# wizyoung/YOLOv3_TensorFlow

Hardware: AMD Instinct MI355X
Metric: images/sec at 416x416 bs=32 (Darknet-53 + 3-scale head forward) (higher is better)
Workload: dtype f32

## Files before the change

yolov3_tensorflow_amd/build.py:

```python
import os
import subprocess
import sys

HERE = os.path.dirname(os.path.abspath(__file__))
CSRC = os.path.join(HERE, "csrc")
LIB = os.path.join(CSRC, "libyolo355.so")

SOURCES = [
    ("y3_abi.hip", []),
    ("y3_net_train.hip", []),
    ("y3_conv.hip", []),
    ("y3_conv_f32s.hip", []),
    ("y3_conv_bf16.hip", []),
    ("y3_conv_bf16x.hip", []),
    ("y3_conv_bf16r.hip", []),
    ("y3_conv_bf16s.hip", []),
    ("y3_conv_bf16b.hip", []),
    ("y3_conv_split.hip", []),
    ("y3_conv_wino.hip", []),
    ("y3_conv_wino44.hip", []),
    ("y3_decode.hip", ["-ffp-contract=off"]),
    ("y3_nms.hip", ["-ffp-contract=off"]),
    ("y3_ops.hip", ["-ffp-contract=off"]),
    ("y3_train.hip", ["-ffp-contract=off"]),
    ("y3_wgrad.hip", []),
    ("y3_wgrad_bf16.hip", []),
    ("y3_wgrad_wino.hip", []),
    ("y3_feed_gpu.hip", ["-ffp-contract=off"]),
    ("y3_jpeg.hip", []),
    ("y3_voc.hip", ["-ffp-contract=off"]),
    ("y3_beval.hip", ["-ffp-contract=off"]),
    ("y3_coco.hip", ["-ffp-contract=off"]),
]
COMMON = ["--offload-arch=gfx950", "-O3", "-std=c++17", "-fPIC", "-Wall", "-Wno-unused-function"]


FEED_SRC = os.path.join(CSRC, "y3_feed.cpp")
JPEG_SRC = os.path.join(CSRC, "y3_jpeg.cpp")
FEED_LIB = os.path.join(CSRC, "liby3feed.so")
FEED_FLAGS = ["-O3", "-std=c++17", "-fPIC", "-shared", "-ffp-contract=off", "-fno-fast-math", "-pthread", "-Wall",
              "-Wno-format-truncation"]


def build_feed(force=False, verbose=True):
    deps = [FEED_SRC, JPEG_SRC, os.path.join(HERE, "..", "include", "yolo355_feed.h"),
            os.path.join(HERE, "..", "include", "yolo355_jpeg.h")]
    if not force and os.path.exists(FEED_LIB) and all(os.path.getmtime(d) <= os.path.getmtime(FEED_LIB) for d in deps):
        return FEED_LIB
    tmp = FEED_LIB + ".%d.tmp" % os.getpid()
    cmd = [os.environ.get("CXX", "g++")] + FEED_FLAGS + [FEED_SRC, JPEG_SRC, "-o", tmp]
    if verbose:
        print(" ".join(cmd), flush=True)
    out = subprocess.run(cmd, stdout=subprocess.PIPE, stderr=subprocess.STDOUT)
    if out.returncode != 0:
        raise RuntimeError("building liby3feed.so failed:\n%s\n%s" % (" ".join(cmd), out.stdout.decode(errors="replace")))
    os.replace(tmp, FEED_LIB)
    return FEED_LIB


def _hipcc():
    for cand in (os.environ.get("HIPCC"), "/opt/rocm/bin/hipcc", "hipcc"):
        if cand and (os.path.isabs(cand) and os.path.exists(cand) or not os.path.isabs(cand)):
            return cand
    raise RuntimeError("hipcc not found")


def csrc_sha16():
    import hashlib
    h = hashlib.sha256()
    names = sorted(n for n in os.listdir(CSRC) if n.endswith(('.hip', '.h')))
    for path in [os.path.join(CSRC, n) for n in names] + [os.path.join(HERE, "..", "include", "yolo355.h")]:
        with open(path, 'rb') as f:
            h.update(os.path.basename(path).encode() + b'\0' + f.read())
    return h.hexdigest()[:16]


def needs_build():
    if not os.path.exists(LIB):
        return True
    t = os.path.getmtime(LIB)
    headers = sorted(n for n in os.listdir(CSRC) if n.endswith('.h'))
    deps = [os.path.join(CSRC, s) for s, _ in SOURCES] + [os.path.join(CSRC, n) for n in headers] + [
        os.path.join(HERE, "..", "include", "yolo355_jpeg.h"),
        os.path.join(HERE, "..", "include", "yolo355_feed.h"),
        os.path.join(HERE, "..", "include", "yolo355.h"),
        os.path.abspath(__file__),
    ]
    return any(os.path.getmtime(d) > t for d in deps if os.path.exists(d))


EXP_LIB = os.path.join(CSRC, "libyolo355_exp.so")
EXP_SOURCES = ("y3_conv.hip", "y3_conv_f32s.hip", "y3_conv_bf16x.hip", "y3_conv_bf16r.hip", "y3_conv_bf16s.hip", "y3_conv_bf16b.hip", "y3_conv_split.hip", "y3_conv_wino.hip", "y3_conv_wino44.hip")


def build_experiments(verbose=True):
    build(verbose=verbose)
    deps = [os.path.join(CSRC, s) for s in EXP_SOURCES] + [LIB]
    if os.path.exists(EXP_LIB) and all(os.path.getmtime(d) <= os.path.getmtime(EXP_LIB) for d in deps):
        return EXP_LIB
    hipcc = _hipcc()
    procs, objs = [], []
    for src, extra in SOURCES:
        obj = os.path.join(CSRC, src.replace(".hip", ".o"))
        if src in EXP_SOURCES:
            obj = os.path.join(CSRC, src.replace(".hip", ".exp.o"))
            cmd = [hipcc] + COMMON + extra + ["-DY3_EXPERIMENTS", "-c", os.path.join(CSRC, src), "-o", obj]
            if verbose:
                print(" ".join(cmd), flush=True)
            procs.append((cmd, subprocess.Popen(cmd, stdout=subprocess.PIPE, stderr=subprocess.STDOUT)))
        objs.append(obj)
    for cmd, p in procs:
        out, _ = p.communicate()
        if p.returncode != 0:
            raise RuntimeError("hipcc failed:\n%s\n%s" % (" ".join(cmd), out.decode(errors="replace")))
    subprocess.check_call([hipcc, "--offload-arch=gfx950", "-shared", "-fPIC", "-o", EXP_LIB] + objs)
    return EXP_LIB


def build(force=False, verbose=True):
    build_feed(force=force, verbose=verbose)
    if not force and not needs_build():
        return LIB
    hipcc = _hipcc()
    objs = []
    procs = []
    for src, extra in SOURCES:
        path = os.path.join(CSRC, src)
        if not os.path.exists(path):
            continue
        obj = os.path.join(CSRC, src.replace(".hip", ".o"))
        cmd = [hipcc] + COMMON + extra + ["-c", path, "-o", obj]
        if verbose:
            print(" ".join(cmd), flush=True)
        procs.append((cmd, subprocess.Popen(cmd, stdout=subprocess.PIPE, stderr=subprocess.STDOUT)))
        objs.append(obj)
    for cmd, p in procs:
        out, _ = p.communicate()
        if p.returncode != 0:
            raise RuntimeError("hipcc failed:\n%s\n%s" % (" ".join(cmd), out.decode(errors="replace")))
        if verbose and out.strip():
            print(out.decode(errors="replace"))
    cmd = [hipcc, "--offload-arch=gfx950", "-shared", "-fPIC", "-o", LIB] + objs
    if verbose:
        print(" ".join(cmd), flush=True)
    subprocess.check_call(cmd)
    return LIB


if __name__ == "__main__":
    build(force="--force" in sys.argv)
    print(LIB)
    if "--experiments" in sys.argv:
        print(build_experiments())
```

yolov3_tensorflow_amd/csrc/y3_conv_wino.hip:

```cpp
#include <cstdlib>
#include <type_traits>
#include "y3_lds.h"

namespace {

struct WinoArgs {
    const float* x;
    const float* u;
    const float* scale;
    const float* shift;
    const float* resid;
    float* y;
    int N, H, W, Cin, Cout, act;
    int TH, TW, T;
    float* partial;
    unsigned* flags;
    int workers;
    unsigned* err;
    unsigned spin_limit;
    int fault;
    float* stats;
    int hybrid;
    int bn_inner;
};

__device__ __host__ __forceinline__ long long wk_begin(long long items, int workers, int w) {
    const long long q = items / workers, r = items % workers;
    return (long long)w * q + (w < r ? w : r);
}

__device__ __host__ __forceinline__ void wk_range(int blocks, int ksteps, int workers, int x, int j, int hybrid,
                                                  long long& begin, long long& end, int* rounds = nullptr,
                                                  int* first_block = nullptr) {
    const int G = workers >> 3;
    const long long b0 = wk_begin(blocks, 8, x), b1 = wk_begin(blocks, 8, x + 1);
    const int R = hybrid ? (int)((b1 - b0) / G) : 0;
    const long long s0 = b0 + (long long)R * G;
    const long long items = (b1 - s0) * ksteps;
    begin = s0 * ksteps + wk_begin(items, G, j);
    end = s0 * ksteps + wk_begin(items, G, j + 1);
    if (rounds) *rounds = R;
    if (first_block) *first_block = (int)b0 + j;
}

typedef __attribute__((address_space(1))) unsigned gu32;

constexpr int WKC = 8;
constexpr int WROW = 32;

__device__ __forceinline__ int opaque(int v) {
    asm volatile("" : "+v"(v));
    return v;
}

__device__ __forceinline__ int lds_off(int row, int half) { return row * WROW + ((half ^ ((row >> 3) & 1)) << 4); }

template <int BT, int BNW, int NT = 256, bool TWO = false>
struct WinoRows {
    static constexpr int LDC = BNW + 4;
    static constexpr int C4 = BNW / 4;
    static constexpr int RPP = NT / C4;
    static constexpr int PASSES = BT * 4 / RPP;
    static_assert(PASSES <= 32, "one validity bit per pass");
    unsigned off[PASSES];
    unsigned ok;
    f32x4 res[PASSES];

    __device__ __forceinline__ void prepare(const WinoArgs& p, const int* tile_pix, const int* tile_ok, int n0) {
        const int tid = opaque(threadIdx.x);
        const int co = n0 + (tid % C4) * 4, tr = tid / C4;
        const bool cok = co < p.Cout;
        ok = 0;
        const __amdgpu_buffer_rsrc_t rs = __builtin_amdgcn_make_buffer_rsrc(
            const_cast<float*>(p.resid), 0, p.resid ? (unsigned)((size_t)p.N * p.H * p.W * p.Cout * 4) : 0u, 0x00020000);
#pragma unroll
        for (int i = 0; i < PASSES; ++i) {
            const int rr = tr + i * RPP;
            const int tl = rr >> 2, q = rr & 3;
            const int pix = tile_pix[tl];
            const int tok = tile_ok[tl];
            const bool oki = cok & (((tok >> q) & 1) != 0);
            ok |= (oki ? 1u : 0u) << i;
            off[i] = (unsigned)(pix + (q >> 1) * p.W + (q & 1)) * (unsigned)p.Cout + (unsigned)co;
            res[i] = __builtin_bit_cast(f32x4, __builtin_amdgcn_raw_buffer_load_b128(rs, oki ? off[i] * 4u : OOB, 0, 0));
        }
    }

    template <bool STATS = false, typename F>
    __device__ __forceinline__ void finish(const WinoArgs& p, const float* cs, int n0, F between,
                                           int n_extra = 0, unsigned extra_base = 0, f32x4* s1 = nullptr,
                                           f32x4* s2 = nullptr) const {
        const int tid = threadIdx.x;
        const int tc = (tid % C4) * 4, tr = tid / C4;
        const int co = n0 + tc;
        f32x4 sc = {0.f, 0.f, 0.f, 0.f}, sh = {0.f, 0.f, 0.f, 0.f};
        if (co < p.Cout) {
            sc = *reinterpret_cast<const f32x4*>(p.scale + co);
            sh = *reinterpret_cast<const f32x4*>(p.shift + co);
        }
        const __amdgpu_buffer_rsrc_t rs_x = __builtin_amdgcn_make_buffer_rsrc(
            p.partial, 0, n_extra ? (unsigned)((size_t)p.workers * BT * 4 * BNW * 4) : 0u, 0x00020000);
        const __amdgpu_buffer_rsrc_t rs_y = __builtin_amdgcn_make_buffer_rsrc(
            p.y, 0, (unsigned)((size_t)p.N * p.H * p.W * p.Cout * 4), 0x00020000);
#pragma unroll
        for (int i = 0; i < PASSES; ++i) {
            f32x4 v = *reinterpret_cast<const f32x4*>(cs + (tr + i * RPP) * LDC + tc);
            if (TWO) v += *reinterpret_cast<const f32x4*>(cs + (BT * 4 + tr + i * RPP) * LDC + tc);
            for (int e = 0; e < n_extra; ++e)
                v += __builtin_bit_cast(f32x4, __builtin_amdgcn_raw_buffer_load_b128(
                         rs_x, (unsigned)((tr + i * RPP) * BNW + tc) * 4u,
                         extra_base + (unsigned)e * (unsigned)(BT * 4 * BNW * 4), 17));
            v = v * sc + sh;
            if (p.act) {
#pragma unroll
                for (int q = 0; q < 4; ++q) v[q] = v[q] > 0.f ? v[q] : 0.1f * v[q];
            }
            v += res[i];
            __builtin_amdgcn_raw_buffer_store_b128(__builtin_bit_cast(u32x4, v), rs_y,
                                                   ((ok >> i) & 1) ? off[i] * 4u : OOB, 0, 0);
            if (STATS) {
                const float m = ((ok >> i) & 1) ? 1.f : 0.f;
                *s1 += v * m;
                *s2 += (v * v) * m;
            }
            between(i);
        }
    }
};

__device__ __forceinline__ int fastdiv(int t, int d) {
    int q = (int)((float)t * __frcp_rn((float)d));
    const int r = t - q * d;
    q += (r >= d) ? 1 : 0;
    q -= (r < 0) ? 1 : 0;
    return q;
}

__device__ __forceinline__ void wino_tile_info(const WinoArgs& p, int t, int& pix, int& okbits, int& n, int& ty,
                                               int& tx) {
    n = ty = tx = 0;
    pix = -1;
    okbits = 0;
    if (t < p.T) {
        n = fastdiv(t, p.TH * p.TW);
        const int rem = t - n * p.TH * p.TW;
        ty = fastdiv(rem, p.TW);
        tx = rem - ty * p.TW;
        pix = (n * p.H + 2 * ty) * p.W + 2 * tx;
        okbits = 1 | ((2 * tx + 1 < p.W) ? 2 : 0) | ((2 * ty + 1 < p.H) ? 4 : 0) |
                 ((2 * tx + 1 < p.W && 2 * ty + 1 < p.H) ? 8 : 0);
    }
}

template <bool STREAMK, bool STATS = false>
__global__ void __launch_bounds__(512, 1) conv_wino8_f32_kernel(const WinoArgs p) {
    constexpr int BT = 64, BNW = 64, NT = 512;
    constexpr int PLANE_V = BT * WROW, PLANE_U = BNW * WROW;
    constexpr int STAGE_V = 16 * PLANE_V, STAGE_U = 16 * PLANE_U;
    constexpr int LDC = BNW + 4;
    constexpr int CS_BYTES = BT * 4 * LDC * 4;
    static_assert(2 * CS_BYTES >= 2 * (STAGE_V + STAGE_U), "the tile tables sit behind the two staging tiles");

    extern __shared__ __attribute__((aligned(16))) unsigned char smem[];
    unsigned char* Vs = smem;
    unsigned char* Us = smem + 2 * STAGE_V;
    int* tile_pix = reinterpret_cast<int*>(smem + 2 * CS_BYTES);
    int* tile_ok = tile_pix + BT;

    const int tid = threadIdx.x, lane = tid & 63, wave = tid >> 6;
    const int ph = wave >> 2, wm = (wave >> 1) & 1, wn = wave & 1;
    const int nbt = (p.T + BT - 1) / BT;
    const int ksteps = p.Cin / WKC;
    long long item, item_end;
    int worker = 0, grp = 0, lw = 0;
    int dp_left = 0, dp_blk = 0;
    const int nbn_ = (p.Cout + BNW - 1) / BNW;
    const int nblocks = nbt * nbn_;
    {
        const int nt = gridDim.x;
        const int q8 = nt >> 3, r8 = nt & 7, xcd = blockIdx.x & 7, k8 = blockIdx.x >> 3;
        const int id = (xcd < r8 ? xcd * (q8 + 1) : r8 * (q8 + 1) + (xcd - r8) * q8) + k8;
        if (STREAMK) {
            grp = xcd;
            lw = (p.workers >> 3) - 1 - k8;
            worker = grp * (p.workers >> 3) + lw;
            wk_range(nblocks, ksteps, p.workers, grp, lw, p.hybrid, item, item_end, &dp_left, &dp_blk);
        } else {
            item = (long long)id * ksteps;
            item_end = item + ksteps;
        }
    }
    if (dp_left == 0 && item >= item_end) return;
    const int first_blk = dp_left > 0 ? dp_blk : (int)(item / ksteps);
    const int first_ks = dp_left > 0 ? 0 : (int)(item - (long long)first_blk * ksteps);

    const __amdgpu_buffer_rsrc_t rs_x = __builtin_amdgcn_make_buffer_rsrc(
        const_cast<float*>(p.x), 0, (unsigned)((size_t)p.N * p.H * p.W * p.Cin * 4), 0x00020000);
    const __amdgpu_buffer_rsrc_t rs_u = __builtin_amdgcn_make_buffer_rsrc(
        const_cast<float*>(p.u), 0, (unsigned)((size_t)16 * p.Cin * p.Cout * 4), 0x00020000);
    unsigned voff_a[12];
    unsigned voff_u[4];
    const int a_tile = (tid & 255) >> 2, a_pair = tid & 3, a_half = tid >> 8;
    int t0 = 0, n0 = 0;
    auto setup_tables = [&](int blk) {
        int bn, bt;
        if (p.bn_inner) { bt = fastdiv(blk, nbn_); bn = blk - bt * nbn_; }
        else            { bn = fastdiv(blk, nbt); bt = blk - bn * nbt; }
        t0 = bt * BT;
        n0 = bn * BNW;
        if (a_pair == 0 && a_half == 0) {
            int pix, okbits, n, ty, tx;
            wino_tile_info(p, t0 + a_tile, pix, okbits, n, ty, tx);
            tile_pix[a_tile] = pix;
            tile_ok[a_tile] = okbits;
        }
    };
    auto setup_voff = [&](int blk) {
        int bn, bt;
        if (p.bn_inner) { bt = fastdiv(blk, nbn_); bn = blk - bt * nbn_; }
        else            { bn = fastdiv(blk, nbt); bt = blk - bn * nbt; }
        const int t0 = bt * BT, n0 = bn * BNW;
        const int tid = opaque(threadIdx.x);
        {
            const int a_tile = (tid & 255) >> 2, a_pair = tid & 3, a_half = tid >> 8;
            int pix, okbits, n, ty, tx;
            wino_tile_info(p, t0 + a_tile, pix, okbits, n, ty, tx);
            const bool tok = pix >= 0;
            const int y0 = 2 * ty - 1 + a_half, x0 = 2 * tx - 1;
#pragma unroll
            for (int i = 0; i < 3; ++i)
#pragma unroll
                for (int j = 0; j < 4; ++j) {
                    const int yy = y0 + i, xx = x0 + j;
                    const bool ok = tok && (unsigned)yy < (unsigned)p.H && (unsigned)xx < (unsigned)p.W;
                    voff_a[i * 4 + j] = ok ? (unsigned)(((n * p.H + yy) * p.W + xx) * p.Cin + a_pair * 2) * 4u : OOB;
                }
        }
#pragma unroll
        for (int j = 0; j < 4; ++j) {
            const int q = tid + NT * j;
            const int pos = q / (2 * BNW), co = (q >> 1) % BNW, half = q & 1;
            const bool ok = (n0 + co) < p.Cout;
            voff_u[j] = ok ? (unsigned)(((size_t)pos * ksteps * p.Cout + (n0 + co)) * WKC + half * 4) * 4u : OOB;
        }
    };
    f32x2 ra[12];
    f32x4 ru[4];
    auto issue = [&](int ks) {
        const unsigned soff_a = (unsigned)(ks * WKC) * 4u;
        const unsigned soff_u = (unsigned)((size_t)ks * p.Cout * WKC) * 4u;
#pragma unroll
        for (int j = 0; j < 12; ++j)
            ra[j] = __builtin_bit_cast(f32x2, __builtin_amdgcn_raw_buffer_load_b64(rs_x, voff_a[j], soff_a, 0));
#pragma unroll
        for (int j = 0; j < 4; ++j)
            ru[j] = __builtin_bit_cast(f32x4, __builtin_amdgcn_raw_buffer_load_b128(rs_u, voff_u[j], soff_u, 0));
    };
    const int st_a = lds_off(a_tile, a_pair >> 1) + (a_pair & 1) * 8;
    auto store = [&](int buf, auto half_c) {
        constexpr int HALF = decltype(half_c)::value;
        unsigned char* us = Us + buf * STAGE_U;
#pragma unroll
        for (int j = 0; j < 4; ++j) {
            const int q = tid + NT * j;
            const int pos = q / (2 * BNW), co = (q >> 1) % BNW, half = q & 1;
            *reinterpret_cast<f32x4*>(us + pos * PLANE_U + lds_off(co, half)) = ru[j];
        }
        f32x2 x[4], y[4];
#pragma unroll
        for (int j = 0; j < 4; ++j) {
            x[j] = ra[0 * 4 + j] - ra[2 * 4 + j];
            y[j] = HALF ? ra[1 * 4 + j] - ra[0 * 4 + j] : ra[1 * 4 + j] + ra[2 * 4 + j];
        }
        unsigned char* vx = Vs + buf * STAGE_V + st_a + (HALF ? 12 : 0) * PLANE_V;
        unsigned char* vy = Vs + buf * STAGE_V + st_a + (HALF ? 8 : 4) * PLANE_V;
        *reinterpret_cast<f32x2*>(vx + 0 * PLANE_V) = x[0] - x[2];
        *reinterpret_cast<f32x2*>(vx + 1 * PLANE_V) = x[1] + x[2];
        *reinterpret_cast<f32x2*>(vx + 2 * PLANE_V) = x[2] - x[1];
        *reinterpret_cast<f32x2*>(vx + 3 * PLANE_V) = x[1] - x[3];
        *reinterpret_cast<f32x2*>(vy + 0 * PLANE_V) = y[0] - y[2];
        *reinterpret_cast<f32x2*>(vy + 1 * PLANE_V) = y[1] + y[2];
        *reinterpret_cast<f32x2*>(vy + 2 * PLANE_V) = y[2] - y[1];
        *reinterpret_cast<f32x2*>(vy + 3 * PLANE_V) = y[1] - y[3];
    };

    f32x16 acc[8];
#pragma unroll
    for (int pos = 0; pos < 8; ++pos)
#pragma unroll
        for (int r = 0; r < 16; ++r) acc[pos][r] = 0.f;

    const int frag_a = lds_off(wm * 32 + (lane & 31), lane >> 5) + ph * 8 * PLANE_V;
    const int frag_b = lds_off(wn * 32 + (lane & 31), lane >> 5) + ph * 8 * PLANE_U;
    auto frags = [&](int buf, int g, f32x4 (&a)[2], f32x4 (&b)[2]) {
        const unsigned char* vs = Vs + buf * STAGE_V + frag_a;
        const unsigned char* us = Us + buf * STAGE_U + frag_b;
#pragma unroll
        for (int i = 0; i < 2; ++i) {
            a[i] = *reinterpret_cast<const f32x4*>(vs + (g * 2 + i) * PLANE_V);
            b[i] = *reinterpret_cast<const f32x4*>(us + (g * 2 + i) * PLANE_U);
        }
    };
    auto mfmas = [&](int g, const f32x4 (&a)[2], const f32x4 (&b)[2], int j0, int j1) {
#pragma unroll
        for (int j = j0; j < j1; ++j)
#pragma unroll
            for (int i = 0; i < 2; ++i)
                acc[g * 2 + i] = __builtin_amdgcn_mfma_f32_32x32x2f32(a[i][j], b[i][j], acc[g * 2 + i], 0, 0, 0);
    };
    f32x4 a0[2], b0[2];

    float* cs = reinterpret_cast<float*>(smem);
    setup_voff(first_blk);
    issue(first_ks);
    while (dp_left > 0 || item < item_end) {
        const bool whole = STREAMK && dp_left > 0;
        const int blk = whole ? dp_blk : (int)(item / ksteps);
        const int ks0 = whole ? 0 : (int)(item - (long long)blk * ksteps);
        const long long blk_end = (long long)(blk + 1) * ksteps;
        const long long seg_end = whole ? item : (blk_end < item_end ? blk_end : item_end);
        const int ks1 = whole ? ksteps : ks0 + (int)(seg_end - item);
        const bool whole_next = whole && dp_left > 1;
        const bool has_next = whole_next || seg_end < item_end;
        const int next_blk = whole_next ? blk + (p.workers >> 3) : (int)(seg_end / ksteps);
        const int next_ks = whole_next ? 0 : (int)(seg_end - (long long)next_blk * ksteps);
        setup_tables(blk);
        if (ph) store(0, std::integral_constant<int, 1>());
        else store(0, std::integral_constant<int, 0>());
        __syncthreads();
        frags(0, 0, a0, b0);
#define W8_WEAVE(TAIL)                                                   \
    do {                                                                 \
        _Pragma("unroll") for (int i = 0; i < 8; ++i) {                  \
            __builtin_amdgcn_sched_group_barrier(0x008, 1, 0);           \
            __builtin_amdgcn_sched_group_barrier(0x020, 2, 0);           \
            if (i >= 4) __builtin_amdgcn_sched_group_barrier(0x100, 1, 0); \
        }                                                                \
        _Pragma("unroll") for (int i = 0; i < 16; ++i) {                 \
            __builtin_amdgcn_sched_group_barrier(0x008, 1, 0);           \
            if ((i & 7) >= 4) __builtin_amdgcn_sched_group_barrier(0x100, 1, 0); \
        }                                                                \
        __builtin_amdgcn_sched_group_barrier(0x008, TAIL, 0);            \
    } while (0)
        if (ph && ks0 + 1 < ks1) issue(ks0 + 1);
        for (int ks = ks0; ks + 1 < ks1; ++ks) {
            const int cur = (ks - ks0) & 1;
            f32x4 a1[2], b1[2];
            if (ph == 0) {
                issue(ks + 1);
                frags(cur, 1, a1, b1);
                mfmas(0, a0, b0, 0, 4);
                frags(cur, 2, a0, b0);
                mfmas(1, a1, b1, 0, 4);
                frags(cur, 3, a1, b1);
                mfmas(2, a0, b0, 0, 4);
                mfmas(3, a1, b1, 0, 2);
                W8_WEAVE(4);
                __builtin_amdgcn_sched_barrier(0);
                store(cur ^ 1, std::integral_constant<int, 0>());
                __builtin_amdgcn_sched_barrier(0);
                __syncthreads();
                frags(cur ^ 1, 0, a0, b0);
                mfmas(3, a1, b1, 2, 4);
            } else {
                store(cur ^ 1, std::integral_constant<int, 1>());
                __builtin_amdgcn_sched_barrier(0);
                issue(ks + 2 < ks1 ? ks + 2 : ks + 1);
                frags(cur, 1, a1, b1);
                mfmas(0, a0, b0, 0, 4);
                frags(cur, 2, a0, b0);
                mfmas(1, a1, b1, 0, 4);
                frags(cur, 3, a1, b1);
                mfmas(2, a0, b0, 0, 4);
                mfmas(3, a1, b1, 0, 4);
                W8_WEAVE(8);
                __builtin_amdgcn_sched_barrier(0);
                __syncthreads();
                frags(cur ^ 1, 0, a0, b0);
            }
        }
        {
            const int cur = (ks1 - 1 - ks0) & 1;
            f32x4 a1[2], b1[2];
#pragma unroll
            for (int g = 0; g < 4; ++g) {
                if (g < 3) frags(cur, g + 1, a1, b1);
                mfmas(g, a0, b0, 0, 4);
#pragma unroll
                for (int i = 0; i < 2; ++i) { a0[i] = a1[i]; b0[i] = b1[i]; }
            }
        }

        __syncthreads();
        const bool producer = STREAMK && ks0 > 0;
        WinoRows<BT, BNW, NT, true> rows;
        rows.prepare(p, tile_pix, tile_ok, n0);
        {
            const int col = wn * 32 + (lane & 31);
            float* csh = cs + ph * (BT * 4 * LDC);
#pragma unroll
            for (int r = 0; r < 16; ++r) {
                const int tl = wm * 32 + (r & 3) + 8 * (r >> 2) + 4 * (lane >> 5);
                float m[8];
#pragma unroll
                for (int pos = 0; pos < 8; ++pos) {
                    m[pos] = acc[pos][r];
                }
                float s0[4], s1[4];
#pragma unroll
                for (int j = 0; j < 4; ++j) {
                    s0[j] = ph ? m[j] : m[j] + m[4 + j];
                    s1[j] = ph ? -m[j] - m[4 + j] : m[4 + j];
                }
                float* row = csh + (tl * 4) * LDC + col;
                row[0 * LDC] = s0[0] + s0[1] + s0[2];
                row[1 * LDC] = s0[1] - s0[2] - s0[3];
                row[2 * LDC] = s1[0] + s1[1] + s1[2];
                row[3 * LDC] = s1[1] - s1[2] - s1[3];
            }
        }
        __syncthreads();
        int n_extra = 0;
        if (STREAMK && ks1 < ksteps) {
            const int G = p.workers >> 3;
            for (int jj = lw + 1; jj < G; ++jj) {
                long long b, e;
                wk_range(nblocks, ksteps, p.workers, grp, jj, p.hybrid, b, e);
                if (b >= blk_end) break;
                ++n_extra;
            }
            if (tid == 0) {
                for (int e = 0; e < n_extra; ++e) {
                    gu32* flag = (gu32*)(p.flags + worker + 1 + e);
                    unsigned spins = 0;
                    for (; spins < p.spin_limit; ++spins) {
                        if (__hip_atomic_load(flag, __ATOMIC_RELAXED, __HIP_MEMORY_SCOPE_AGENT) != 0u) break;
                        __builtin_amdgcn_s_sleep(8);
                    }
                    if (spins == p.spin_limit && p.err)
                        __hip_atomic_fetch_or(p.err, Y3_ERR_STREAMK_TIMEOUT, __ATOMIC_RELAXED, __HIP_MEMORY_SCOPE_SYSTEM);
                }
                __builtin_amdgcn_fence(__ATOMIC_ACQUIRE, "agent");
            }
            __syncthreads();
        }
        if (STREAMK && has_next) {
            setup_voff(next_blk);
            issue(next_ks);
            __builtin_amdgcn_sched_barrier(0);
        }
        if (!producer) {
            static_assert(WinoRows<BT, BNW, NT, true>::PASSES == 8, "one accumulator set is reset per store pass");
            f32x4 s1 = {0.f, 0.f, 0.f, 0.f}, s2 = {0.f, 0.f, 0.f, 0.f};
            rows.template finish<STATS>(p, cs, n0, [&](int i) {
#pragma unroll
                for (int r = 0; r < 16; ++r) acc[i][r] = 0.f;
            }, n_extra, (unsigned)(worker + 1) * (unsigned)(BT * 4 * BNW * 4), &s1, &s2);
            if (STATS) {
                constexpr int C4 = BNW / 4, RPP = NT / C4;
                const int tc = (tid % C4) * 4, tr = tid / C4;
                __syncthreads();
                float* red = cs;
                *reinterpret_cast<f32x4*>(red + (tr * 2 + 0) * BNW + tc) = s1;
                *reinterpret_cast<f32x4*>(red + (tr * 2 + 1) * BNW + tc) = s2;
                __syncthreads();
                if (tid < C4 && n0 + tc < p.Cout) {
                    f32x4 a = {0.f, 0.f, 0.f, 0.f}, b = {0.f, 0.f, 0.f, 0.f};
#pragma unroll
                    for (int k = 0; k < RPP; ++k) {
                        a += *reinterpret_cast<const f32x4*>(red + (k * 2 + 0) * BNW + tc);
                        b += *reinterpret_cast<const f32x4*>(red + (k * 2 + 1) * BNW + tc);
                    }
                    float* st = p.stats + (size_t)(t0 / BT) * 2 * p.Cout;
                    *reinterpret_cast<f32x4*>(st + n0 + tc) = a;
                    *reinterpret_cast<f32x4*>(st + p.Cout + n0 + tc) = b;
                }
                if (!STREAMK) __syncthreads();
            }
        } else {
#pragma unroll
            for (int pos = 0; pos < 8; ++pos)
#pragma unroll
                for (int r = 0; r < 16; ++r) acc[pos][r] = 0.f;
            const __amdgpu_buffer_rsrc_t rs_part = __builtin_amdgcn_make_buffer_rsrc(
                p.partial, 0, (unsigned)((size_t)p.workers * BT * 4 * BNW * 4), 0x00020000);
            const unsigned slot_off = (unsigned)worker * (unsigned)(BT * 4 * BNW * 4);
            constexpr int C4 = BNW / 4;
            for (int f = tid; f < BT * 4 * C4; f += NT) {
                const int rr = f / C4, c4 = f - rr * C4;
                const f32x4 v = *reinterpret_cast<const f32x4*>(cs + rr * LDC + c4 * 4) +
                                *reinterpret_cast<const f32x4*>(cs + (BT * 4 + rr) * LDC + c4 * 4);
                __builtin_amdgcn_raw_buffer_store_b128(__builtin_bit_cast(u32x4, v), rs_part,
                                                       slot_off + (unsigned)f * 16u, 0, 16);
            }
            asm volatile("s_waitcnt vmcnt(0)" ::: "memory");
            __syncthreads();
            if (tid == 0 && !p.fault)
                __hip_atomic_store((gu32*)(p.flags + worker), 1u, __ATOMIC_RELAXED, __HIP_MEMORY_SCOPE_AGENT);
        }
        if (STREAMK) __syncthreads();
        if (whole) { --dp_left; dp_blk += p.workers >> 3; }
        item = seg_end;
    }
}

__global__ void __launch_bounds__(256) pack_weights_wino_kernel(const float* __restrict__ w_hwio, float* __restrict__ out,
                                                                int cin, int cout, int dgrad) {
    __shared__ float g[9][WKC][33];
    const int tid = threadIdx.x;
    const int ncb = (cout + 31) / 32;
    const int kb = blockIdx.x / ncb, cb = blockIdx.x - kb * ncb;
    const int ci0 = kb * WKC, co0 = cb * 32;
    if (!dgrad) {
        const int col = tid & 31, cil = tid >> 5;
        const bool ok = co0 + col < cout && ci0 + cil < cin;
#pragma unroll
        for (int t = 0; t < 9; ++t)
            g[t][cil][col] = ok ? w_hwio[((size_t)t * cin + ci0 + cil) * cout + co0 + col] : 0.f;
    } else {
        const int cil = tid & 7, col = tid >> 3;
        const bool ok = co0 + col < cout && ci0 + cil < cin;
#pragma unroll
        for (int t = 0; t < 9; ++t)
            g[t][cil][col] = ok ? w_hwio[((size_t)(8 - t) * cout + co0 + col) * cin + ci0 + cil] : 0.f;
    }
    __syncthreads();
    const int cil = tid & 7, col = tid >> 3;
    if (co0 + col >= cout || ci0 + cil >= cin) return;
    float t[4][3];
#pragma unroll
    for (int b = 0; b < 3; ++b) {
        const float g0 = g[0 * 3 + b][cil][col], g1 = g[1 * 3 + b][cil][col], g2 = g[2 * 3 + b][cil][col];
        t[0][b] = g0;
        t[1][b] = 0.5f * (g0 + g1 + g2);
        t[2][b] = 0.5f * (g0 - g1 + g2);
        t[3][b] = g2;
    }
#pragma unroll
    for (int a = 0; a < 4; ++a) {
        const float u[4] = {t[a][0], 0.5f * (t[a][0] + t[a][1] + t[a][2]), 0.5f * (t[a][0] - t[a][1] + t[a][2]),
                            t[a][2]};
#pragma unroll
        for (int b = 0; b < 4; ++b)
            out[(((size_t)(a * 4 + b) * (cin / WKC) + kb) * cout + co0 + col) * WKC + cil] = u[b];
    }
}

}

void y3_wino_range_impl(int units, int ksteps, int workers, int group, int local_worker, int hybrid, long long* begin,
                        long long* end) {
    wk_range(units, ksteps, workers, group, local_worker, hybrid, *begin, *end);
}

int y3_conv_wino_eligible_impl(const y3_conv_desc* d) {
    return d && d->k == 3 && d->stride == 1 && d->c_up == 0 && d->cin % 32 == 0 && d->cout % 32 == 0 &&
           d->n > 0 && d->h > 1 && d->w > 1;
}

int y3_launch_pack_wino(hipStream_t stream, const float* w_hwio, int cin, int cout, float* out, int dgrad) {
    const int blocks = (cin / WKC) * ((cout + 31) / 32);
    hipLaunchKernelGGL(pack_weights_wino_kernel, dim3(blocks), dim3(256), 0, stream, w_hwio, out, cin, cout, dgrad);
    Y3_CHECK_HIP(hipGetLastError());
    return Y3_OK;
}

constexpr int WK_WORKERS = 256;
constexpr int WINO_BT = 64;

int y3_conv_wino_stats_blocks_impl(const y3_conv_desc* d) {
    if (!y3_conv_wino_eligible_impl(d)) return 0;
    const long long T = (long long)d->n * ((d->h + 1) / 2) * ((d->w + 1) / 2);
    return (int)((T + WINO_BT - 1) / WINO_BT);
}

constexpr size_t WK_SLOT_BYTES = (size_t)64 * 4 * 64 * sizeof(float);
constexpr size_t WK_FLAGS_OFFSET = (size_t)WK_WORKERS * WK_SLOT_BYTES;

size_t y3_conv_wino_workspace_bytes_impl(const y3_conv_desc* d) {
    if (!y3_conv_wino_eligible_impl(d)) return 0;
    return WK_FLAGS_OFFSET + (size_t)WK_WORKERS * sizeof(unsigned);
}

int y3_launch_conv_wino(hipStream_t stream, const y3_conv_desc* d, const float* x, const float* u, const float* scale,
                        const float* shift, const float* residual, float* y, void* workspace, size_t workspace_bytes,
                        const y3_sk_opts* sk) {
    Y3_CHECK_ARG(d && x && u && scale && shift && y, "y3_conv2d_fwd_wino: null pointer argument");
    Y3_CHECK_ARG(y3_conv_wino_eligible_impl(d),
                 "y3_conv2d_fwd_wino: needs a 3x3 stride-1 conv with Cin %% 32 == 0, Cout %% 32 == 0 and no "
                 "fused upsample input");
    const long long M = (long long)d->n * d->h * d->w;
    Y3_CHECK_ARG(M * d->cin < (1LL << 29) && M * d->cout < (1LL << 29),
                 "y3_conv2d_fwd_wino: tensor exceeds 2^29 elements (32-bit byte offsets)");
    WinoArgs a;
    a.x = x; a.u = u; a.scale = scale; a.shift = shift; a.resid = residual; a.y = y;
    a.N = d->n; a.H = d->h; a.W = d->w; a.Cin = d->cin; a.Cout = d->cout; a.act = d->act;
    a.TH = (d->h + 1) / 2; a.TW = (d->w + 1) / 2; a.T = d->n * a.TH * a.TW;
    a.partial = nullptr; a.flags = nullptr; a.workers = 0;
    a.err = nullptr; a.spin_limit = 0; a.fault = 0;
    a.stats = sk ? sk->stats : nullptr;
    {
        static int hyb = -1;
        if (hyb < 0) {
            const char* e = y3_exp_env("Y3_WINO_SK_HYBRID");
            hyb = e ? (atoi(e) != 0) : 0;
        }
        a.hybrid = hyb;
    }
    {
        static int force = -2;
        if (force == -2) {
            const char* e = y3_exp_env("Y3_WINO_ORDER");
            force = e ? atoi(e) : -1;
        }
        a.bn_inner = force >= 0 ? (force != 0) : ((size_t)16 * d->cin * d->cout * sizeof(float) <= (size_t)(1u << 20));
    }
    constexpr int BT = WINO_BT, BNW = 64;
    constexpr int workers = WK_WORKERS;
    constexpr size_t lds = (size_t)2 * BT * 4 * (BNW + 4) * sizeof(float) + 2 * BT * sizeof(int);
    const int nbt = (a.T + BT - 1) / BT, nbn = (a.Cout + BNW - 1) / BNW;
    const int blocks = nbt * nbn;
    static int force = -2;
    if (force == -2) {
        const char* e = y3_exp_env("Y3_CONV_WINO_STREAMK");
        force = e ? atoi(e) : -1;
    }
    const bool has_ws = workspace != nullptr && workspace_bytes >= y3_conv_wino_workspace_bytes_impl(d) &&
                        ((uintptr_t)workspace & 15) == 0;
    bool use_sk = has_ws && blocks > workers && blocks < 8 * workers && blocks % workers != 0;
    if (force >= 0) use_sk = has_ws && force != 0 && blocks >= workers;
    if (use_sk) {
        a.partial = static_cast<float*>(workspace);
        a.workers = workers;
        a.err = sk ? sk->err : nullptr;
        y3_sk_debug_env(&a.spin_limit, &a.fault);
        if (sk && sk->flags) {
            a.flags = sk->flags;
        } else {
            a.flags = reinterpret_cast<unsigned*>(static_cast<char*>(workspace) + WK_FLAGS_OFFSET);
            Y3_CHECK_HIP(hipMemsetAsync(a.flags, 0, (size_t)workers * sizeof(unsigned), stream));
        }
        return a.stats ? y3_launch_lds<conv_wino8_f32_kernel<true, true>>(stream, dim3(workers), dim3(512), lds, a)
                       : y3_launch_lds<conv_wino8_f32_kernel<true, false>>(stream, dim3(workers), dim3(512), lds, a);
    }
    return a.stats ? y3_launch_lds<conv_wino8_f32_kernel<false, true>>(stream, dim3(blocks), dim3(512), lds, a)
                   : y3_launch_lds<conv_wino8_f32_kernel<false, false>>(stream, dim3(blocks), dim3(512), lds, a);
}
```

yolov3_tensorflow_amd/csrc/y3_internal.h:

```cpp
#pragma once
#include <hip/hip_runtime.h>
#include <stdint.h>
#include <stddef.h>
#include "../../include/yolo355.h"

struct y3_ctx {
    int device;
    hipStream_t stream;
    unsigned* err_host;
    void* stage_host = nullptr;
    size_t stage_bytes = 0;
    hipEvent_t stage_ev = nullptr;
    bool stage_busy = false;
};
int y3_ctx_stage_acquire(y3_ctx* ctx, size_t bytes, void** out);
int y3_ctx_stage_release(y3_ctx* ctx);
int ctx_pending_error(const y3_ctx* ctx);

struct y3_sk_opts {
    unsigned* flags = nullptr;
    unsigned* err = nullptr;
    float* stats = nullptr;
    const float* bwd_z = nullptr;
    const float* bwd_vec = nullptr;
    int wino44_form = -1;
};
int y3_conv_stats_blocks_impl(const y3_conv_desc* d, int wino);
int y3_conv_dgrad_stats_blocks_impl(const y3_conv_desc* fwd);
#define Y3_ERR_STREAMK_TIMEOUT 1u
void y3_sk_debug_env(unsigned* spin_limit, int* fault);

constexpr long long Y3_CONV_RANGE_LIMIT = 1LL << 29;
constexpr int Y3_MAX_RANGES = 256;
long long y3_conv_range_limit();
int y3_conv_image_ranges_impl(const y3_conv_desc* d, int dz_stride, long long limit, int max_ranges, int* begin, int* count);
struct y3_image_ranges {
    int n = 0;
    int begin[Y3_MAX_RANGES], count[Y3_MAX_RANGES];
    y3_image_ranges(const y3_conv_desc* d, int dz_stride) {
        n = y3_conv_image_ranges_impl(d, dz_stride, y3_conv_range_limit(), Y3_MAX_RANGES, begin, count);
    }
};

#ifdef Y3_EXPERIMENTS
#include <cstdlib>
static inline const char* y3_exp_env(const char* name) { return getenv(name); }
#else
static inline const char* y3_exp_env(const char*) { return nullptr; }
#endif

void y3_set_error(const char* fmt, ...);

constexpr int Y3_MAX_DEVICES = 16;
int y3_current_device();
size_t y3_device_max_lds();

#define Y3_CHECK_ARG(cond, ...)                \
    do {                                       \
        if (!(cond)) {                         \
            y3_set_error(__VA_ARGS__);         \
            return Y3_EINVAL;                  \
        }                                      \
    } while (0)

#define Y3_CHECK_HIP(expr)                                                          \
    do {                                                                            \
        hipError_t e_ = (expr);                                                     \
        if (e_ != hipSuccess) {                                                     \
            y3_set_error("%s failed: %s (%s:%d)", #expr, hipGetErrorString(e_),     \
                         __FILE__, __LINE__);                                       \
            return Y3_EHIP;                                                         \
        }                                                                           \
    } while (0)

template <auto Kern, typename... Args>
int y3_launch_lds(hipStream_t stream, dim3 grid, dim3 block, size_t lds, const Args&... args) {
    static bool attr_set[Y3_MAX_DEVICES] = {};
    const int dev = y3_current_device();
    if (dev < 0 || !attr_set[dev]) {
        Y3_CHECK_HIP(hipFuncSetAttribute(reinterpret_cast<const void*>(Kern), hipFuncAttributeMaxDynamicSharedMemorySize, (int)lds));
        if (dev >= 0) attr_set[dev] = true;
    }
    hipLaunchKernelGGL(Kern, grid, block, lds, stream, args...);
    Y3_CHECK_HIP(hipGetLastError());
    return Y3_OK;
}
inline int y3_blocks_for(size_t total, int cap = 4096) { return (int)((total + 255) / 256 < (size_t)cap ? (total + 255) / 256 : (size_t)cap); }

typedef float f32x4 __attribute__((ext_vector_type(4)));
typedef f32x4 f32x4_u __attribute__((aligned(4)));
typedef float f32x16 __attribute__((ext_vector_type(16)));

int y3_launch_conv(hipStream_t stream, const y3_conv_desc* d, const float* x, const float* x_up,
                   const float* w, const float* scale, const float* shift, const float* residual,
                   float* y, void* workspace, size_t workspace_bytes, const y3_sk_opts* sk = nullptr);
size_t y3_conv_workspace_bytes_impl(const y3_conv_desc* d);
int y3_conv_schedule_impl(const y3_conv_desc* d);
int y3_conv_schedule_query(const y3_conv_desc* conv, int tmode_taps, int with_workspace);
int y3_streamk_range_impl(int kind, int units, int ksteps, int workers, int group, int local_worker, long long* begin,
                          long long* end);
void y3_wino_range_impl(int units, int ksteps, int workers, int group, int local_worker, int hybrid, long long* begin,
                        long long* end);
int y3_launch_conv_dgrad(hipStream_t stream, const y3_conv_desc* fwd, const float* dz, int dz_stride,
                         const float* w_d, const float* ones, const float* zeros, int accumulate, float* dx,
                         void* workspace, size_t workspace_bytes, const y3_sk_opts* sk = nullptr);
int y3_launch_conv_bf16(hipStream_t stream, const y3_conv_desc* d, const void* x, const void* x_up, const void* w,
                        const float* scale, const float* shift, const void* residual, void* y, int out_f32);
int y3_conv_bf16_train_stats_blocks(const y3_conv_desc* d);
int y3_launch_conv_bf16_train(hipStream_t stream, const y3_conv_desc* d, const void* x, const void* w, void* z, float* stats);
int y3_launch_conv_bf16_reg(hipStream_t stream, const y3_conv_desc* d, const void* x, const void* w, const float* scale,
                            const float* shift, void* y, int out_f32);
int y3_launch_conv_bf16_dgrad(hipStream_t stream, const y3_conv_desc* fwd, const void* dz, int dz_stride, const void* w_d,
                              int accumulate, float* dx);
int y3_pack_conv_weights_bf16_reg(y3_ctx* ctx, const float* w_hwio, int k, int cin, int cout, int dgrad_stride, void* w_packed);
int y3_launch_conv_wgrad_bf16(hipStream_t stream, const y3_conv_desc* d, const void* x, const void* dz, int dz_stride, float* dw,
                              void* scratch, size_t scratch_bytes);
int y3_conv_bf16x_takes(int k, int cin);
int y3_launch_pack_bf16x(hipStream_t stream, const float* w_hwio, int k, int cin, int cout, void* w_packed);
int y3_launch_conv_bf16x(hipStream_t stream, const y3_conv_desc* d, const void* x, const void* x_up, const void* w,
                         const float* scale, const float* shift, const void* residual, void* y, int out_f32);
int y3_conv_f32_stem_s2_takes(const y3_conv_desc* d0, const y3_conv_desc* d1);
int y3_launch_conv_f32_stem_s2(hipStream_t stream, int n, int h, int w, const float* x, const float* w0, const float* scale0,
                               const float* shift0, int act0, const float* w1_packed, const float* scale1, const float* shift1,
                               int act1, float* y);
int y3_conv_bf16_stem_s2_takes(const y3_conv_desc* d0, const y3_conv_desc* d1);
int y3_launch_conv_bf16_stem_s2(hipStream_t stream, int n, int h, int w, const float* x, const float* w0, const float* scale0,
                                const float* shift0, int act0, const void* w1_packed, const float* scale1, const float* shift1,
                                int act1, void* y);
int y3_conv_bf16_resblock64_takes(const y3_conv_desc* d2, const y3_conv_desc* d3);
int y3_launch_conv_bf16_resblock64(hipStream_t stream, int n, int h, int w, const void* x, const void* w2_packed,
                                   const float* scale2, const float* shift2, int act2, const void* w3_packed, const float* scale3,
                                   const float* shift3, int act3, void* y);
int y3_conv_bf16r_takes(int k, int cin);
int y3_conv_bf16r_tile(const y3_conv_desc* d);
int y3_launch_conv_bf16r(hipStream_t stream, const y3_conv_desc* d, const void* x, const void* x_up, const void* w,
                         const float* scale, const float* shift, const void* residual, void* y, int out_f32);
int y3_launch_pack_split(hipStream_t stream, const float* w_hwio, int k, int cin, int cout, int planes, void* out,
                         int transposed = 0);
int y3_launch_conv_dgrad_split(hipStream_t stream, const y3_conv_desc* fwd, int planes, const float* dz, int dz_stride,
                               const void* w, const float* ones, const float* zeros, int accumulate, float* dx,
                               void* workspace, size_t workspace_bytes, const y3_sk_opts* sk = nullptr);
int y3_launch_conv_split(hipStream_t stream, const y3_conv_desc* d, int planes, const float* x, const float* x_up,
                         const void* w, const float* scale, const float* shift, const float* residual, float* y,
                         void* workspace, size_t workspace_bytes, const y3_sk_opts* sk = nullptr);
int y3_conv_wino_eligible_impl(const y3_conv_desc* d);
int y3_conv_wino_stats_blocks_impl(const y3_conv_desc* d);
int y3_conv_wino44_eligible_impl(const y3_conv_desc* d);
int y3_conv_wino44_candidate_impl(const y3_conv_desc* d);
int y3_conv_wino44_preferred_impl(const y3_conv_desc* d);
int y3_launch_pack_wino44(hipStream_t stream, const float* w_hwio, int cin, int cout, float* out, int dgrad = 0);
int y3_conv_wino44_stats_blocks_impl(const y3_conv_desc* d);
size_t y3_conv_wino44_workspace_bytes_impl(const y3_conv_desc* d);
int y3_conv_wino44_two_pass_impl(const y3_conv_desc* d);
int y3_launch_conv_wino44(hipStream_t stream, const y3_conv_desc* d, const float* x, const float* u, const float* scale,
                          const float* shift, const float* residual, float* y, void* workspace, size_t workspace_bytes,
                          const y3_sk_opts* sk);
int y3_launch_wgrad_sum_splits(hipStream_t stream, const float* scratch, int nsplit, long long n4, float* dw);
int y3_conv_wgrad_wino_eligible_impl(const y3_conv_desc* d);
size_t y3_conv_wgrad_wino_scratch_bytes_impl(const y3_conv_desc* d);
int y3_launch_conv_wgrad_wino(hipStream_t stream, const y3_conv_desc* d, const float* x, const float* dz, int dz_stride,
                              float* dw_hwio, void* scratch, size_t scratch_bytes);
int y3_launch_pack_wino(hipStream_t stream, const float* w_hwio, int cin, int cout, float* out, int dgrad = 0);
size_t y3_conv_wino_workspace_bytes_impl(const y3_conv_desc* d);
int y3_launch_conv_wino(hipStream_t stream, const y3_conv_desc* d, const float* x, const float* u, const float* scale,
                        const float* shift, const float* residual, float* y, void* workspace, size_t workspace_bytes,
                        const y3_sk_opts* sk = nullptr);
```

Measured before the change: 3396.

## Add persistent Winograd F(2,3) kernel specialized for Cin=32 Cout=64 conv

Adds a dedicated persistent Winograd kernel for the 3x3 conv with 32 input and 64 output channels, the first residual block at 208x208. Each block of two half-groups keeps the transformed filter in registers and double-buffers input patches in LDS via async DMA. It overlaps the output transform, residual add and stores of one tile with the input DMA and MFMA work for the next. The kernel is dispatched by default when stats are not requested, in place of the generic Winograd path, which was a poor fit for such a small channel count. It adds a specialized code path with hand-managed barriers and a fixed 256-block grid.

Measured after the change: 3392. About the same (-0.1%).

```diff
diff --git a/yolov3_tensorflow_amd/build.py b/yolov3_tensorflow_amd/build.py
--- a/yolov3_tensorflow_amd/build.py
+++ b/yolov3_tensorflow_amd/build.py
@@ -18,6 +18,7 @@
     ("y3_conv_bf16b.hip", []),
     ("y3_conv_split.hip", []),
     ("y3_conv_wino.hip", []),
+    ("y3_conv_wino_c32.hip", []),
     ("y3_conv_wino44.hip", []),
     ("y3_decode.hip", ["-ffp-contract=off"]),
     ("y3_nms.hip", ["-ffp-contract=off"]),
@@ -90,7 +91,7 @@
 
 
 EXP_LIB = os.path.join(CSRC, "libyolo355_exp.so")
-EXP_SOURCES = ("y3_conv.hip", "y3_conv_f32s.hip", "y3_conv_bf16x.hip", "y3_conv_bf16r.hip", "y3_conv_bf16s.hip", "y3_conv_bf16b.hip", "y3_conv_split.hip", "y3_conv_wino.hip", "y3_conv_wino44.hip")
+EXP_SOURCES = ("y3_conv.hip", "y3_conv_f32s.hip", "y3_conv_bf16x.hip", "y3_conv_bf16r.hip", "y3_conv_bf16s.hip", "y3_conv_bf16b.hip", "y3_conv_split.hip", "y3_conv_wino.hip", "y3_conv_wino_c32.hip", "y3_conv_wino44.hip")
 
 
 def build_experiments(verbose=True):
diff --git a/yolov3_tensorflow_amd/csrc/y3_conv_wino.hip b/yolov3_tensorflow_amd/csrc/y3_conv_wino.hip
--- a/yolov3_tensorflow_amd/csrc/y3_conv_wino.hip
+++ b/yolov3_tensorflow_amd/csrc/y3_conv_wino.hip
@@ -600,6 +600,15 @@
     a.err = nullptr; a.spin_limit = 0; a.fault = 0;
     a.stats = sk ? sk->stats : nullptr;
     {
+        static int c32 = -2;
+        if (c32 == -2) {
+            const char* e = y3_exp_env("Y3_WINO_C32");
+            c32 = e ? atoi(e) : -1;
+        }
+        if (c32 != 0 && !a.stats && y3_conv_wino_c32_takes(d))
+            return y3_launch_conv_wino_c32(stream, d, x, u, scale, shift, residual, y);
+    }
+    {
         static int hyb = -1;
         if (hyb < 0) {
             const char* e = y3_exp_env("Y3_WINO_SK_HYBRID");
diff --git a/yolov3_tensorflow_amd/csrc/y3_conv_wino_c32.hip b/yolov3_tensorflow_amd/csrc/y3_conv_wino_c32.hip
--- /dev/null
+++ b/yolov3_tensorflow_amd/csrc/y3_conv_wino_c32.hip
@@ -0,0 +1,214 @@
+#include "y3_lds.h"
+
+namespace {
+
+struct C32Args {
+    const float* x;
+    const float* u;
+    const float* scale;
+    const float* shift;
+    const float* resid;
+    float* y;
+    int N, H, W, act;
+    int RH, RW;
+    int items;
+    int rounds;
+};
+
+constexpr int CIN = 32, COUT = 64;
+constexpr int IH = 4, IW = 16;
+constexpr int PH = IH + 2, PW = IW + 2;
+constexpr int CHUNKS = PH * PW * (CIN / 4);
+constexpr int RAW_BYTES = 4 * 256 * 16;
+constexpr int VSTR = CIN + 4;
+constexpr int V_POS = 16 * VSTR * 4;
+constexpr int V_BYTES = 16 * V_POS;
+constexpr int ST_BYTES = IH * IW * 16 * 4;
+constexpr int OFF_V = 2 * RAW_BYTES;
+constexpr int OFF_ST = OFF_V + 2 * V_BYTES;
+constexpr int C32_LDS = OFF_ST + 8 * ST_BYTES;
+static_assert(CHUNKS <= 4 * 256, "four DMA rounds cover the patch");
+
+__device__ __forceinline__ void phase_barrier() {
+    asm volatile("s_waitcnt lgkmcnt(0)" ::: "memory");
+    __builtin_amdgcn_s_barrier();
+    asm volatile("" ::: "memory");
+}
+
+__global__ void __launch_bounds__(512, 1) conv_wino_c32_f32_kernel(const C32Args p) {
+    extern __shared__ __attribute__((aligned(16))) unsigned char smem[];
+    const int tid = threadIdx.x, lane = tid & 63;
+    const int wave = __builtin_amdgcn_readfirstlane(tid >> 6);
+    const int half = wave >> 2, cq = wave & 3;
+    const int th = tid & 255;
+    unsigned char* raw = smem + half * RAW_BYTES;
+    unsigned char* V = smem + OFF_V + half * V_BYTES;
+    float* st = reinterpret_cast<float*>(smem + OFF_ST + wave * ST_BYTES);
+
+    const unsigned x_bytes = (unsigned)((size_t)p.N * p.H * p.W * CIN * 4);
+    const unsigned y_bytes = (unsigned)((size_t)p.N * p.H * p.W * COUT * 4);
+    const __amdgpu_buffer_rsrc_t rs_x = __builtin_amdgcn_make_buffer_rsrc(const_cast<float*>(p.x), 0, x_bytes, 0x00020000);
+    const __amdgpu_buffer_rsrc_t rs_r =
+        __builtin_amdgcn_make_buffer_rsrc(const_cast<float*>(p.resid), 0, p.resid ? y_bytes : 0u, 0x00020000);
+    const __amdgpu_buffer_rsrc_t rs_y = __builtin_amdgcn_make_buffer_rsrc(p.y, 0, y_bytes, 0x00020000);
+
+    const int G = 2 * (int)gridDim.x, g = 2 * (int)blockIdx.x + half;
+
+    f32x4 uu[32];
+    {
+        const float* up = p.u + ((size_t)((lane >> 4) * COUT + cq * 16 + (lane & 15))) * 8;
+#pragma unroll
+        for (int pos = 0; pos < 16; ++pos) {
+            uu[pos * 2 + 0] = *reinterpret_cast<const f32x4*>(up + (size_t)pos * (CIN / 8) * COUT * 8);
+            uu[pos * 2 + 1] = *reinterpret_cast<const f32x4*>(up + (size_t)pos * (CIN / 8) * COUT * 8 + 4);
+        }
+    }
+
+    unsigned voff[4];
+    auto patch_offsets = [&](int it) {
+        const bool valid = it < p.items;
+        const int itc = valid ? it : 0;
+        const int n = itc / (p.RH * p.RW), rem = itc - n * (p.RH * p.RW);
+        const int ry = rem / p.RW, rx = rem - ry * p.RW;
+        const int y0 = ry * IH - 1, x0 = rx * IW - 1;
+#pragma unroll
+        for (int q = 0; q < 4; ++q) {
+            const int c = th + 256 * q;
+            const int row = c / (PW * 8), w = c - row * (PW * 8);
+            const int yy = y0 + row, xx = x0 + (w >> 3);
+            const bool ok = valid && c < CHUNKS && (unsigned)yy < (unsigned)p.H && (unsigned)xx < (unsigned)p.W;
+            voff[q] = ok ? (unsigned)(((n * p.H + yy) * p.W + xx) * CIN + (w & 7) * 4) * 4u : OOB;
+        }
+    };
+    auto patch_dma = [&]() {
+#pragma unroll
+        for (int q = 0; q < 4; ++q) dma16(rs_x, raw + q * 4096 + cq * 1024, voff[q], 0);
+    };
+
+    f32x4 acc[16];
+#pragma unroll
+    for (int pos = 0; pos < 16; ++pos) acc[pos] = f32x4{0.f, 0.f, 0.f, 0.f};
+
+    patch_offsets(g);
+    patch_dma();
+    __builtin_amdgcn_s_waitcnt(0x0F70);
+    phase_barrier();
+    if (half) phase_barrier();
+
+    const float slope = p.act ? 0.1f : 1.f;
+    const float sc1 = p.scale[cq * 16 + (lane & 15)], sh1 = p.shift[cq * 16 + (lane & 15)];
+    unsigned ooff[IH] = {OOB, OOB, OOB, OOB};
+    for (int k = 0; k <= p.rounds; ++k) {
+        const int it = g + k * G;
+
+        {
+            f32x4 s0[4], s1[4];
+#pragma unroll
+            for (int b = 0; b < 4; ++b) {
+                s0[b] = acc[0 + b] + acc[4 + b] + acc[8 + b];
+                s1[b] = acc[4 + b] - acc[8 + b] - acc[12 + b];
+            }
+            f32x4 yv[4];
+            yv[0] = s0[0] + s0[1] + s0[2];
+            yv[1] = s0[1] - s0[2] - s0[3];
+            yv[2] = s1[0] + s1[1] + s1[2];
+            yv[3] = s1[1] - s1[2] - s1[3];
+            float* o = st + ((2 * (lane >> 5)) * IW + 8 * ((lane >> 4) & 1)) * 16 + (lane & 15);
+#pragma unroll
+            for (int e = 0; e < 4; ++e) {
+                f32x4 v = yv[e] * sc1 + sh1;
+                const f32x4 vs = v * slope;
+#pragma unroll
+                for (int r = 0; r < 4; ++r) {
+                    float* q = o + ((e >> 1) * IW + 2 * r + (e & 1)) * 16;
+                    *q += fmaxf(v[r], vs[r]);
+                }
+            }
+        }
+#pragma unroll
+        for (int i = 0; i < IH; ++i) {
+            const f32x4 o = *reinterpret_cast<const f32x4*>(st + i * (IW * 16) + lane * 4);
+            __builtin_amdgcn_raw_buffer_store_b128(__builtin_bit_cast(u32x4, o), rs_y, ooff[i], 0, 0);
+        }
+        {
+            const bool valid = it < p.items;
+            const int itc = valid ? it : 0;
+            const int n = itc / (p.RH * p.RW), rem = itc - n * (p.RH * p.RW);
+            const int ry = rem / p.RW, rx = rem - ry * p.RW;
+            const int xx = rx * IW + (lane >> 2);
+#pragma unroll
+            for (int i = 0; i < IH; ++i) {
+                const int yy = ry * IH + i;
+                const bool ok = valid && yy < p.H && xx < p.W;
+                ooff[i] = ok ? (unsigned)(((n * p.H + yy) * p.W + xx) * COUT + cq * 16 + (lane & 3) * 4) * 4u : OOB;
+            }
+        }
+        {
+            const int cp = th & 15, tile = th >> 4, ty = tile >> 3, tx = tile & 7;
+            const unsigned char* src = raw + (((2 * ty) * PW + 2 * tx) * CIN + 2 * cp) * 4;
+            f32x2 d[16], v[16];
+#pragma unroll
+            for (int i = 0; i < 4; ++i)
+#pragma unroll
+                for (int j = 0; j < 4; ++j)
+                    d[i * 4 + j] = *reinterpret_cast<const f32x2*>(src + ((i * PW + j) * CIN) * 4);
+            input_transform(d, v);
+            unsigned char* dst = V + tile * (VSTR * 4) + cp * 8;
+#pragma unroll
+            for (int pos = 0; pos < 16; ++pos) *reinterpret_cast<f32x2*>(dst + pos * V_POS) = v[pos];
+        }
+        patch_offsets(it + G);
+        phase_barrier();
+
+        patch_dma();
+#pragma unroll
+        for (int i = 0; i < IH; ++i) dma16(rs_r, reinterpret_cast<unsigned char*>(st) + i * 1024, ooff[i], 0);
+        {
+            const unsigned char* va = V + (lane & 15) * (VSTR * 4) + (lane >> 4) * 32;
+            f32x4 fr[2][4];
+            auto frags = [&](int pp, f32x4 (&f)[4]) {
+                f[0] = *reinterpret_cast<const f32x4*>(va + (2 * pp) * V_POS);
+                f[1] = *reinterpret_cast<const f32x4*>(va + (2 * pp) * V_POS + 16);
+                f[2] = *reinterpret_cast<const f32x4*>(va + (2 * pp + 1) * V_POS);
+                f[3] = *reinterpret_cast<const f32x4*>(va + (2 * pp + 1) * V_POS + 16);
+            };
+            frags(0, fr[0]);
+#pragma unroll
+            for (int pp = 0; pp < 8; ++pp) {
+                if (pp + 1 < 8) frags(pp + 1, fr[(pp + 1) & 1]);
+                const f32x4 (&f)[4] = fr[pp & 1];
+                f32x4 c0 = {0.f, 0.f, 0.f, 0.f}, c1 = {0.f, 0.f, 0.f, 0.f};
+#pragma unroll
+                for (int j = 0; j < 8; ++j) {
+                    c0 = __builtin_amdgcn_mfma_f32_16x16x4f32(f[j >> 2][j & 3], uu[4 * pp + (j >> 2)][j & 3], c0, 0, 0, 0);
+                    c1 = __builtin_amdgcn_mfma_f32_16x16x4f32(f[2 + (j >> 2)][j & 3], uu[4 * pp + 2 + (j >> 2)][j & 3], c1, 0, 0, 0);
+                }
+                acc[2 * pp] = c0;
+                acc[2 * pp + 1] = c1;
+                __builtin_amdgcn_sched_barrier(0);
+            }
+        }
+        __builtin_amdgcn_s_waitcnt(0x0F70);
+        phase_barrier();
+    }
+    if (!half) phase_barrier();
+}
+
+}
+
+int y3_conv_wino_c32_takes(const y3_conv_desc* d) {
+    return d->cin == CIN && d->cout == COUT && y3_device_max_lds() >= (size_t)C32_LDS;
+}
+
+int y3_launch_conv_wino_c32(hipStream_t stream, const y3_conv_desc* d, const float* x, const float* u, const float* scale,
+                            const float* shift, const float* residual, float* y) {
+    C32Args a;
+    a.x = x; a.u = u; a.scale = scale; a.shift = shift; a.resid = residual; a.y = y;
+    a.N = d->n; a.H = d->h; a.W = d->w; a.act = d->act;
+    a.RH = (d->h + IH - 1) / IH; a.RW = (d->w + IW - 1) / IW;
+    a.items = d->n * a.RH * a.RW;
+    constexpr int workers = 256;
+    const int grid = (a.items + 1) / 2 < workers ? (a.items + 1) / 2 : workers;
+    a.rounds = (a.items + 2 * grid - 1) / (2 * grid);
+    return y3_launch_lds<conv_wino_c32_f32_kernel>(stream, dim3(grid), dim3(512), (size_t)C32_LDS, a);
+}
diff --git a/yolov3_tensorflow_amd/csrc/y3_internal.h b/yolov3_tensorflow_amd/csrc/y3_internal.h
--- a/yolov3_tensorflow_amd/csrc/y3_internal.h
+++ b/yolov3_tensorflow_amd/csrc/y3_internal.h
@@ -145,6 +145,9 @@
                          void* workspace, size_t workspace_bytes, const y3_sk_opts* sk = nullptr);
 int y3_conv_wino_eligible_impl(const y3_conv_desc* d);
 int y3_conv_wino_stats_blocks_impl(const y3_conv_desc* d);
+int y3_conv_wino_c32_takes(const y3_conv_desc* d);
+int y3_launch_conv_wino_c32(hipStream_t stream, const y3_conv_desc* d, const float* x, const float* u, const float* scale,
+                            const float* shift, const float* residual, float* y);
 int y3_conv_wino44_eligible_impl(const y3_conv_desc* d);
 int y3_conv_wino44_candidate_impl(const y3_conv_desc* d);
 int y3_conv_wino44_preferred_impl(const y3_conv_desc* d);
```
